# venetanji/videosd

Measured on AMD Instinct MI355X. Metric: frames/sec (whole node) + p50 per-frame latency, SD1.5 512x512 LCM 4-step, higher is better.
Workload: dtype f16 (fp32 accumulate); 1 GPU; 5 frames per launch x 4 launch lanes in flight (a stream's independent frames coalesced along GEMM M; the batch=1-per-launch figures of a --full run are fps_one_frame_per_launch and p50_latency_ms) of SD1.5 512x512 LCM 4-step img2img, every frame denoised independently, ControlNet-canny + TAESD (BASELINE configs[1], reference-faithful: the reference always runs ControlNet); frames_per_rank=411, frames_per_launch=5, launches_in_flight_per_gpu=4, kernel_launches_per_graph_replay=1430

## Files before the change

videosd_amd/csrc/attention.hip:

```cpp
#include <stdarg.h>
#include <stdlib.h>

#include <type_traits>

#include "common.h"

namespace {

struct AttnParams {
  const half_t* q;
  const half_t* k;
  const half_t* vt;
  half_t* out;
  int ldq, ldk, ldvt, ldo;
  int sq, sk, heads, d;
  float scale_log2;
  int causal;
  int k_brows, vt_bcols;
  VSD_CUT_FIELD
#ifdef VSD_ATTN_PROBE
  long long* probe;
#endif
};

#ifdef VSD_ATTN_PROBE
long long* g_probe = nullptr;
#define PROBE(I_)                                          \
  {                                                        \
    long long t_ = __builtin_readcyclecounter();           \
    pacc[I_] += t_ - plast;                                \
    plast = t_;                                            \
  }
#else
#define PROBE(I_)
#endif

constexpr float NEG_BIG = -1.0e30f;

#ifndef VSD_ATTN_PV_PRIO
#define VSD_ATTN_PV_PRIO 3
#endif

__device__ __forceinline__ float xhalf_max(float x) {
  auto r = __builtin_amdgcn_permlane32_swap(__float_as_uint(x), __float_as_uint(x), false, false);
  return fmaxf(__uint_as_float(r[0]), __uint_as_float(r[1]));
}

constexpr float LAZY_T = 5.0f;
template <int NQK, int NPV, int NW, int QB, int KSP, bool LAZY = false>
__device__ __forceinline__ void attention_body(const AttnParams& pp, const unsigned image) {
  VSD_CUT(VSD_CUT_ATTENTION, pp.cut)
  constexpr int NTG = 64 * NW;
  constexpr int KS = NQK * 16 + 8;
  constexpr int VS = 64 + 8;
  constexpr int DV = NPV * 32;
  constexpr int KTILE = 64 * KS, VTILE = DV * VS;
  constexpr int GROUP_HALFS = 2 * (KTILE + VTILE);
  constexpr int KCH = (64 * NQK * 2 + NTG - 1) / NTG;
  constexpr int VCH = (DV * 8 + NTG - 1) / NTG;
  constexpr int MERGE_FLOATS = KSP > 1 ? NW * QB * (NPV * 16 + 2) * 64 : 0;
  constexpr int SMEM_HALFS = (KSP * GROUP_HALFS > 2 * MERGE_FLOATS) ? KSP * GROUP_HALFS : 2 * MERGE_FLOATS;
  __shared__ __attribute__((aligned(16))) half_t smem[SMEM_HALFS];

  AttnParams p = pp;
  {
    const size_t b = image;
    p.q += b * p.sq * p.ldq;
    p.out += b * p.sq * p.ldo;
    p.k += b * p.k_brows * p.ldk;
    p.vt += b * p.vt_bcols;
  }
  const int tid = threadIdx.x;
  const int lane = tid & 63;
  const int wave = tid >> 6;
  const int grp = wave / NW;
  const int gwave = wave - grp * NW;
  const int gtid = tid - grp * NTG;
  const int lr = lane & 31;
  const int lh = lane >> 5;
  const int head = blockIdx.x;
  const int qblk = blockIdx.y;
  const int q0 = qblk * (32 * NW * QB) + gwave * (32 * QB);
  const int d = p.d;
  const int dch = d >> 3;
  half_t* Ks = smem + grp * GROUP_HALFS;
  half_t* Vs = Ks + 2 * KTILE;

  for (int i = tid; i < KSP * GROUP_HALFS / 8; i += NTG * KSP) reinterpret_cast<u32x4*>(smem)[i] = (u32x4){0u, 0u, 0u, 0u};
  const bool ones_row = d < DV;

  unsigned kg[KCH];
  int kl[KCH], krow[KCH];
#pragma unroll
  for (int i = 0; i < KCH; ++i) {
    int c = gtid + i * NTG;
    bool ok = c < 64 * dch;
    int kr = ok ? c / dch : 0, kc = ok ? c - kr * dch : 0;
    krow[i] = ok ? kr : 1 << 28;
    kg[i] = ok ? (unsigned)(kr * p.ldk + head * d + kc * 8) : 0u;
    kl[i] = kr * KS + kc * 8;
  }
  unsigned vg[VCH];
  int vl[VCH];
  bool vok[VCH];
#pragma unroll
  for (int i = 0; i < VCH; ++i) {
    int c = gtid + i * NTG;
    vok[i] = c < d * 8;
    int vr = vok[i] ? c >> 3 : 0, vc = c & 7;
    vg[i] = vok[i] ? (unsigned)((head * d + vr) * p.ldvt + vc * 8) : 0u;
    vl[i] = vr * VS + (vc >> 1) * 16 + (vc & 1) * 4;
  }
  u32x4 kreg[2][KCH], vreg[2][VCH];
#define ATT_LOAD_K(SET_, KEY0_)                                                                     \
  {                                                                                                 \
    const half_t* kb_ = p.k + (size_t)(KEY0_) * p.ldk;                                              \
    if ((KEY0_) + 64 <= p.sk) {                                                                     \
      _Pragma("unroll") for (int i = 0; i < KCH; ++i) kreg[SET_][i] = *reinterpret_cast<const u32x4*>(kb_ + kg[i]); \
    } else {                                                                                        \
      _Pragma("unroll") for (int i = 0; i < KCH; ++i) {                                             \
        const bool ok = (KEY0_) + krow[i] < p.sk;                                                   \
        kreg[SET_][i] = *reinterpret_cast<const u32x4*>(ok ? kb_ + kg[i] : p.k);                    \
      }                                                                                             \
    }                                                                                               \
  }
#define ATT_LOAD_V(SET_, KEY0_)                                                                     \
  {                                                                                                 \
    const half_t* vb_ = p.vt + (KEY0_);                                                             \
    _Pragma("unroll") for (int i = 0; i < VCH; ++i) vreg[SET_][i] = *reinterpret_cast<const u32x4*>(vb_ + vg[i]); \
  }
#define ATT_STORE_K(SET_, BUF_)                                                                     \
  {                                                                                                 \
    _Pragma("unroll") for (int i = 0; i < KCH; ++i)                                                 \
      if (krow[i] < 64) *reinterpret_cast<u32x4*>(Ks + (BUF_) * KTILE + kl[i]) = kreg[SET_][i];     \
  }
#define ATT_STORE_V(SET_, BUF_)                                                                     \
  {                                                                                                 \
    _Pragma("unroll") for (int i = 0; i < VCH; ++i)                                                 \
      if (vok[i]) {                                                                                 \
        half_t* dst = Vs + (BUF_) * VTILE + vl[i];                                                  \
        *reinterpret_cast<u32x2*>(dst) = (u32x2){vreg[SET_][i][0], vreg[SET_][i][1]};               \
        *reinterpret_cast<u32x2*>(dst + 8) = (u32x2){vreg[SET_][i][2], vreg[SET_][i][3]};           \
      }                                                                                             \
  }
#define ATT_LOAD(SET_, KEY0_) { ATT_LOAD_K(SET_, KEY0_) ATT_LOAD_V(SET_, KEY0_) }
#define ATT_STORE(SET_, BUF_) { ATT_STORE_K(SET_, BUF_) ATT_STORE_V(SET_, BUF_) }

  half8 qf[QB][NQK];
  int qrow[QB];
  bool qvalid[QB];
#pragma unroll
  for (int qb = 0; qb < QB; ++qb) {
    qrow[qb] = q0 + 32 * qb + lr;
    qvalid[qb] = qrow[qb] < p.sq;
#pragma unroll
    for (int ks = 0; ks < NQK; ++ks) {
      int doff = ks * 16 + lh * 8;
      half8 v = (half8){0, 0, 0, 0, 0, 0, 0, 0};
      if (qvalid[qb] && doff < d) {
        v = *reinterpret_cast<const half8*>(p.q + (size_t)qrow[qb] * p.ldq + head * d + doff);
#pragma unroll
        for (int j = 0; j < 8; ++j) v[j] = (half_t)((float)v[j] * p.scale_log2);
      }
      qf[qb][ks] = v;
    }
  }

  f32x16 o[QB][NPV];
  float m_run[QB], l_run[QB];
#pragma unroll
  for (int qb = 0; qb < QB; ++qb) {
    m_run[qb] = NEG_BIG;
    l_run[qb] = 0.f;
#pragma unroll
    for (int i = 0; i < NPV; ++i)
#pragma unroll
      for (int r = 0; r < 16; ++r) o[qb][i][r] = 0.f;
  }

  [[maybe_unused]] bool lazy_first = true;
  if constexpr (LAZY) {
#pragma unroll
    for (int qb = 0; qb < QB; ++qb) m_run[qb] = 0.f;
  }
  int sk_end = p.sk;
  if (p.causal) sk_end = min(p.sk, qblk * (32 * NW * QB) + 32 * NW * QB);
  const int ntiles = (sk_end + 63) / 64;
  const int niter = (ntiles + KSP - 1) / KSP;

  auto slot_key0 = [&](int j) { return (j * KSP + grp) * 64; };
  auto slot_ok = [&](int j) { return j * KSP + grp < ntiles; };
#ifdef VSD_ATTN_PROBE
  long long pacc[8] = {0, 0, 0, 0, 0, 0, 0, 0};
  long long plast = __builtin_readcyclecounter();
#endif
  auto qk_tile = [&](const int buf, f32x16 (&s)[QB][2]) __attribute__((always_inline)) {
      const half_t* Kb = Ks + buf * KTILE;
#pragma unroll
      for (int kb = 0; kb < 2; ++kb)
#pragma unroll
        for (int qb = 0; qb < QB; ++qb)
#pragma unroll
          for (int r = 0; r < 16; ++r) s[qb][kb][r] = 0.f;
#pragma unroll
      for (int ks = 0; ks < NQK; ++ks) {
#pragma unroll
        for (int kb = 0; kb < 2; ++kb) {
          half8 kf = *reinterpret_cast<const half8*>(Kb + (kb * 32 + lr) * KS + ks * 16 + lh * 8);
#pragma unroll
          for (int qb = 0; qb < QB; ++qb) s[qb][kb] = __builtin_amdgcn_mfma_f32_32x32x16_f16(kf, qf[qb][ks], s[qb][kb], 0, 0, 0);
        }
      }
      PROBE(1)
      __builtin_amdgcn_s_setprio(0);
  };
  auto softmax_pv = [&](const int buf, const int key0, auto masked, f32x16 (&s)[QB][2]) __attribute__((always_inline)) {
      const half_t* Vb = Vs + buf * VTILE;
      if constexpr (decltype(masked)::value) {
#pragma unroll
        for (int qb = 0; qb < QB; ++qb)
#pragma unroll
          for (int kb = 0; kb < 2; ++kb)
#pragma unroll
            for (int r = 0; r < 16; ++r) {
              int key = key0 + kb * 32 + (r & 3) + 8 * (r >> 2) + 4 * lh;
              bool ok = key < p.sk && (!p.causal || key <= qrow[qb]);
              if (!ok) s[qb][kb][r] = NEG_BIG;
            }
      }
      if constexpr (LAZY) {
        float mx[QB];
        bool need = false;
#pragma unroll
        for (int qb = 0; qb < QB; ++qb) {
          float v = NEG_BIG;
#pragma unroll
          for (int kb = 0; kb < 2; ++kb)
#pragma unroll
            for (int r = 0; r < 16; ++r) v = fmaxf(v, s[qb][kb][r]);
          mx[qb] = xhalf_max(v);
          need = need || mx[qb] > LAZY_T;
        }
        const bool moved = __builtin_amdgcn_ballot_w64(need) != 0;
        if (lazy_first || moved) {
#pragma unroll
          for (int qb = 0; qb < QB; ++qb) {
            const bool mine = lazy_first || mx[qb] > LAZY_T;
            float m_new = mine ? fminf(fmaxf(m_run[qb] + mx[qb], -60000.f), 60000.f) : m_run[qb];
            m_new = (float)(half_t)m_new;
            const float delta = m_new - m_run[qb];
            const float alpha = __builtin_amdgcn_exp2f(-delta);
#pragma unroll
            for (int kb = 0; kb < 2; ++kb)
#pragma unroll
              for (int r = 0; r < 16; ++r) s[qb][kb][r] = __builtin_amdgcn_exp2f(s[qb][kb][r] - delta);
            if (!lazy_first) {
#pragma unroll
              for (int i = 0; i < NPV; ++i)
#pragma unroll
                for (int r = 0; r < 16; ++r) o[qb][i][r] *= alpha;
            }
            m_run[qb] = m_new;
            if (lh == 1) qf[qb][NQK - 1][0] = (half_t)(-m_new);
          }
          lazy_first = false;
        } else {
#pragma unroll
          for (int qb = 0; qb < QB; ++qb)
#pragma unroll
            for (int kb = 0; kb < 2; ++kb)
#pragma unroll
              for (int r = 0; r < 16; ++r) s[qb][kb][r] = __builtin_amdgcn_exp2f(s[qb][kb][r]);
        }
      } else {
      bool grew_any = false;
      float alpha[QB];
#pragma unroll
      for (int qb = 0; qb < QB; ++qb) {
        float mx = NEG_BIG;
#pragma unroll
        for (int kb = 0; kb < 2; ++kb)
#pragma unroll
          for (int r = 0; r < 16; ++r) mx = fmaxf(mx, s[qb][kb][r]);
        mx = xhalf_max(mx);
        const float m_new = fmaxf(m_run[qb], mx);
        grew_any = grew_any || (m_new > m_run[qb]);
        alpha[qb] = __builtin_amdgcn_exp2f(m_run[qb] - m_new);
        m_run[qb] = m_new;
        if (ones_row) {
#pragma unroll
          for (int kb = 0; kb < 2; ++kb)
#pragma unroll
            for (int r = 0; r < 16; ++r) s[qb][kb][r] = __builtin_amdgcn_exp2f(s[qb][kb][r] - m_new);
        } else {
          float psum = 0.f;
#pragma unroll
          for (int kb = 0; kb < 2; ++kb)
#pragma unroll
            for (int r = 0; r < 16; ++r) {
              float e = __builtin_amdgcn_exp2f(s[qb][kb][r] - m_new);
              s[qb][kb][r] = e;
              psum += e;
            }
          l_run[qb] = l_run[qb] * alpha[qb] + psum;
        }
      }
      if (__builtin_amdgcn_ballot_w64(grew_any) != 0) {
#pragma unroll
        for (int qb = 0; qb < QB; ++qb)
#pragma unroll
          for (int i = 0; i < NPV; ++i)
#pragma unroll
            for (int r = 0; r < 16; ++r) o[qb][i][r] *= alpha[qb];
      }
      }

      PROBE(2)
      __builtin_amdgcn_s_setprio(VSD_ATTN_PV_PRIO);
#pragma unroll
      for (int kb = 0; kb < 2; ++kb) {
#pragma unroll
        for (int st = 0; st < 2; ++st) {
          half8 pf[QB];
#pragma unroll
          for (int qb = 0; qb < QB; ++qb)
#pragma unroll
            for (int j = 0; j < 8; ++j) pf[qb][j] = (half_t)s[qb][kb][8 * st + j];
#pragma unroll
          for (int db = 0; db < NPV; ++db) {
            half8 vf = *reinterpret_cast<const half8*>(Vb + (db * 32 + lr) * VS + kb * 32 + 16 * st + 8 * lh);
#pragma unroll
            for (int qb = 0; qb < QB; ++qb) o[qb][db] = __builtin_amdgcn_mfma_f32_32x32x16_f16(vf, pf[qb], o[qb][db], 0, 0, 0);
          }
        }
      }
      PROBE(3)
  };
  auto run_softmax_pv = [&](int j, const int buf, f32x16 (&s)[QB][2]) __attribute__((always_inline)) {
    const int key0 = slot_key0(j);
    if ((key0 + 64 > p.sk) || p.causal) softmax_pv(buf, key0, std::true_type{}, s);
    else softmax_pv(buf, key0, std::false_type{}, s);
  };

  if (slot_ok(0)) ATT_LOAD(0, slot_key0(0))
  if (slot_ok(1)) ATT_LOAD(1, slot_key0(1))
  __syncthreads();
  if (ones_row && gtid < 2 * 64) Vs[(gtid >> 6) * VTILE + (DV - 1) * VS + (gtid & 63)] = (half_t)1.0f;
  if (LAZY && gtid < 2 * 64) Ks[(gtid >> 6) * KTILE + (gtid & 63) * KS + d] = (half_t)1.0f;
  if (slot_ok(0)) ATT_STORE(0, 0)
  __syncthreads();
  auto run_tile = [&](int j) __attribute__((always_inline)) {
    f32x16 s[QB][2];
    qk_tile(j & 1, s);
    run_softmax_pv(j, j & 1, s);
  };
  for (int it = 0; it < niter; it += 2) {
    if (slot_ok(it + 2)) ATT_LOAD(0, slot_key0(it + 2))
    PROBE(0)
    if (slot_ok(it)) run_tile(it);
    if (slot_ok(it + 1)) ATT_STORE(1, 1)
    PROBE(4)
    __syncthreads();
    PROBE(5)
    if (it + 1 < niter) {
      if (slot_ok(it + 3)) ATT_LOAD(1, slot_key0(it + 3))
      PROBE(0)
      if (slot_ok(it + 1)) run_tile(it + 1);
      if (slot_ok(it + 2)) ATT_STORE(0, 0)
      PROBE(4)
    }
    __syncthreads();
    PROBE(5)
  }
#ifdef VSD_ATTN_PROBE
  if (p.probe && blockIdx.x == 0 && blockIdx.y == 0 && image == 0 && tid == 0)
    for (int i = 0; i < 8; ++i) p.probe[i] = pacc[i];
#endif
#undef ATT_LOAD
#undef ATT_STORE
#undef ATT_LOAD_K
#undef ATT_LOAD_V
#undef ATT_STORE_K
#undef ATT_STORE_V

  if constexpr (KSP > 1) {
    constexpr int PER_WAVE = QB * (NPV * 16 + 2) * 64;
    float* mg = reinterpret_cast<float*>(smem) + gwave * PER_WAVE + lane;
    if (grp == 1) {
#pragma unroll
      for (int qb = 0; qb < QB; ++qb) {
        float* b = mg + qb * (NPV * 16 + 2) * 64;
        b[0] = (LAZY && lazy_first) ? NEG_BIG : m_run[qb];
        b[64] = l_run[qb];
#pragma unroll
        for (int i = 0; i < NPV; ++i)
#pragma unroll
          for (int r = 0; r < 16; ++r) b[(2 + i * 16 + r) * 64] = o[qb][i][r];
      }
    }
    __syncthreads();
    if (grp != 0) return;
#pragma unroll
    for (int qb = 0; qb < QB; ++qb) {
      const float* b = mg + qb * (NPV * 16 + 2) * 64;
      const float m1 = b[0], l1 = b[64];
      const float m = fmaxf(m_run[qb], m1);
      const float a0 = __builtin_amdgcn_exp2f(m_run[qb] - m), a1 = __builtin_amdgcn_exp2f(m1 - m);
      l_run[qb] = l_run[qb] * a0 + l1 * a1;
#pragma unroll
      for (int i = 0; i < NPV; ++i)
#pragma unroll
        for (int r = 0; r < 16; ++r) o[qb][i][r] = o[qb][i][r] * a0 + b[(2 + i * 16 + r) * 64] * a1;
    }
  }

#pragma unroll
  for (int qb = 0; qb < QB; ++qb) {
    float l_tot;
    if (ones_row) {
      const float mine = o[qb][NPV - 1][15];
      const float other = __shfl_xor(mine, 32);
      l_tot = lh ? mine : other;
    } else {
      l_tot = l_run[qb] + __shfl_xor(l_run[qb], 32);
    }
    const float inv = 1.0f / l_tot;
    if (qvalid[qb]) {
      half_t* orow = p.out + (size_t)qrow[qb] * p.ldo + head * d;
#pragma unroll
      for (int db = 0; db < NPV; ++db)
#pragma unroll
        for (int g = 0; g < 4; ++g) {
          int dd = db * 32 + 8 * g + 4 * lh;
          if (dd < d) {
            half4 v;
#pragma unroll
            for (int j = 0; j < 4; ++j) v[j] = (half_t)(o[qb][db][4 * g + j] * inv);
            *reinterpret_cast<half4*>(orow + dd) = v;
          }
        }
    }
  }
}

template <int NQK, int NPV, int NW, int QB, int KSP, bool LAZY = false>
__global__ __launch_bounds__(64 * NW * KSP) void attention_kernel(const AttnParams pp) {
  attention_body<NQK, NPV, NW, QB, KSP, LAZY>(pp, blockIdx.z);
}
template <int NQK, int NPV, int NW, int QB, int KSP>
__global__ __launch_bounds__(64 * NW * KSP) __attribute__((amdgpu_waves_per_eu(3))) void attention_lazy_kernel(const AttnParams pp) {
  attention_body<NQK, NPV, NW, QB, KSP, true>(pp, blockIdx.z);
}
template <int NQK, int NPV, int NW, int QB, int KSP>
__global__ __launch_bounds__(64 * NW * KSP) __attribute__((amdgpu_waves_per_eu(3))) void attention_lazy_pair_kernel(const Pair<AttnParams> g) {
  const unsigned nb = gridDim.z >> 1, which = blockIdx.z >= nb;
  attention_body<NQK, NPV, NW, QB, KSP, true>(g.p[which], blockIdx.z - which * nb);
}
template <int NQK, int NPV, int NW, int QB, int KSP, bool LAZY = false>
__global__ __launch_bounds__(64 * NW * KSP) void attention_pair_kernel(const Pair<AttnParams> g) {
  const unsigned nb = gridDim.z >> 1, which = blockIdx.z >= nb;
  attention_body<NQK, NPV, NW, QB, KSP, LAZY>(g.p[which], blockIdx.z - which * nb);
}

struct AttnShape {
  int nw, qb, ksp;
};

template <int NQK, int NPV, int NW, int QB, int KSP>
void launch_one(vsd_ctx* ctx, const AttnParams& p, int batch, hipStream_t s) {
  dim3 grid(p.heads, (p.sq + 32 * NW * QB - 1) / (32 * NW * QB), batch);
  if constexpr (NQK == 3 && NPV == 2) {
    static const bool off = getenv("VSD_ATTN_NO_LAZY") != nullptr;
    if (p.d == 40 && !p.causal && !off) {
      if constexpr (NW == 4 && KSP == 1)
        launch_pairable(ctx, attention_lazy_kernel<NQK, NPV, NW, QB, KSP>, attention_lazy_pair_kernel<NQK, NPV, NW, QB, KSP>, grid, dim3(64 * NW * KSP), 0, s, p);
      else
        launch_pairable(ctx, attention_kernel<NQK, NPV, NW, QB, KSP, true>, attention_pair_kernel<NQK, NPV, NW, QB, KSP, true>, grid, dim3(64 * NW * KSP), 0, s, p);
      return;
    }
  }
  launch_pairable(ctx, attention_kernel<NQK, NPV, NW, QB, KSP>, attention_pair_kernel<NQK, NPV, NW, QB, KSP>, grid, dim3(64 * NW * KSP), 0, s, p);
}

template <int NQK, int NPV>
void launch_attn(vsd_ctx* ctx, const AttnParams& p, AttnShape sh, int batch, hipStream_t s) {
  constexpr bool SMALL = NPV <= 3;
  if constexpr (SMALL) {
    if (sh.ksp == 2) return launch_one<NQK, NPV, 4, 1, 2>(ctx, p, batch, s);
  }
  if (sh.nw == 2) return launch_one<NQK, NPV, 2, 1, 1>(ctx, p, batch, s);
  return launch_one<NQK, NPV, 4, 1, 1>(ctx, p, batch, s);
}

}

#ifdef VSD_ATTN_PROBE
extern "C" void vsd_attn_set_probe(void* buf) { g_probe = (long long*)buf; }
#endif

extern "C" int vsd_attention(vsd_ctx* ctx, const void* q, int ldq, const void* k, int ldk, const void* vt, int ldvt,
                             void* out, int ldo, int sq, int sk, int heads, int d, float scale, int causal,
                             void* stream) {
  return vsd_attention_batched(ctx, q, ldq, k, ldk, vt, ldvt, out, ldo, sq, sk, heads, d, scale, causal, 1, 0, 0, stream);
}

extern "C" int vsd_attention_batched(vsd_ctx* ctx, const void* q, int ldq, const void* k, int ldk, const void* vt, int ldvt,
                                     void* out, int ldo, int sq, int sk, int heads, int d, float scale, int causal,
                                     int batch, int k_batch_rows, int vt_batch_cols, void* stream) {
  if (!ctx) return VSD_ERR_ARG;
#ifdef VSD_PROBE
  { static const bool skip = getenv("VSD_SKIP_ATTN") != nullptr; if (skip) return VSD_OK; }
#endif
  if (batch < 1 || batch > 65535 || k_batch_rows < 0 || vt_batch_cols < 0 || vt_batch_cols % 8)
    return vsd_fail(ctx, VSD_ERR_ARG, "attention: batch=%d k_batch_rows=%d vt_batch_cols=%d", batch, k_batch_rows, vt_batch_cols);
  if (!q || !k || !vt || !out) return vsd_fail(ctx, VSD_ERR_ARG, "attention: null pointer");
  if (d % 8 || d < 8 || d > 160) return vsd_fail(ctx, VSD_ERR_ARG, "attention: head_dim %d unsupported", d);
  if (sq <= 0 || sk <= 0 || heads <= 0) return vsd_fail(ctx, VSD_ERR_ARG, "attention: empty problem");
  if (ldq % 8 || ldk % 8 || ldvt % 8 || ldo % 4 || ldvt < (batch - 1) * vt_batch_cols + ((sk + 63) / 64) * 64)
    return vsd_fail(ctx, VSD_ERR_ARG, "attention: bad leading dimensions (ldvt=%d must cover round_up(sk=%d,64))", ldvt, sk);
  AttnParams p;
  p.q = (const half_t*)q; p.k = (const half_t*)k; p.vt = (const half_t*)vt; p.out = (half_t*)out;
  p.ldq = ldq; p.ldk = ldk; p.ldvt = ldvt; p.ldo = ldo;
  p.sq = sq; p.sk = sk; p.heads = heads; p.d = d;
  p.scale_log2 = scale * 1.4426950408889634f;
  p.causal = causal;
  p.k_brows = k_batch_rows; p.vt_bcols = vt_batch_cols;
  VSD_CUT_SET(p)
#ifdef VSD_ATTN_PROBE
  p.probe = g_probe;
#endif
  hipStream_t s = (hipStream_t)stream;
  LaunchScope ls(ctx, s, VSD_FAM_ATTENTION, 4.0 * sq * (double)sk * heads * d * batch);
  const int nqk = (d + 15) / 16;
  const long wgs = (long)((sq + 127) / 128) * heads * batch;
  AttnShape sh = {4, 1, 1};
  const int ntiles = (sk + 63) / 64;
  if (d <= 96 && !causal && ntiles >= 8 && wgs <= 256) sh.ksp = 2;
  if (sh.ksp == 1 && wgs < 64) sh.nw = 2;
  if (const char* e = getenv("VSD_ATTN_SHAPE")) {
    int a = 4, b = 1, c = 1;
    if (sscanf(e, "%d,%d,%d", &a, &b, &c) == 3) {
      sh.nw = a == 2 ? 2 : 4;
      sh.qb = 1;
      (void)b;
      sh.ksp = (c == 2 && d <= 96) ? 2 : 1;
    }
  }
  if (nqk <= 1) launch_attn<1, 1>(ctx, p, sh, batch, s);
  else if (nqk == 2) launch_attn<2, 1>(ctx, p, sh, batch, s);
  else if (nqk == 3) launch_attn<3, 2>(ctx, p, sh, batch, s);
  else if (nqk == 4) launch_attn<4, 2>(ctx, p, sh, batch, s);
  else if (nqk == 5) launch_attn<5, 3>(ctx, p, sh, batch, s);
  else if (nqk == 6) launch_attn<6, 3>(ctx, p, sh, batch, s);
  else if (nqk <= 8) launch_attn<8, 4>(ctx, p, sh, batch, s);
  else launch_attn<10, 5>(ctx, p, sh, batch, s);
  return ls.finish();
}
```

Before: 142.4 frames/s.

## Add register-resident short-key attention kernel for cross-attention with few keys

Adds a specialised attention kernel for short key sequences (sk<=96, d<=64, heads<=8), such as the text-conditioning cross-attention with 77 keys. Each wave keeps all K and V fragments for one head in registers, computes the full softmax in a single pass with no online rescaling, and loops over several 32-row query blocks. Each 512-thread block covers all heads, and the next query block is prefetched while the current one is computed. It is chosen automatically when there are enough query blocks to fill the GPU, and trades higher register use and a separate code path for removing repeated K/V loads and the flash-attention bookkeeping.

```diff
diff --git a/videosd_amd/csrc/attention.hip b/videosd_amd/csrc/attention.hip
--- a/videosd_amd/csrc/attention.hip
+++ b/videosd_amd/csrc/attention.hip
@@ -460,6 +460,195 @@
 __global__ __launch_bounds__(64 * NW * KSP) void attention_pair_kernel(const Pair<AttnParams> g) {
   const unsigned nb = gridDim.z >> 1, which = blockIdx.z >= nb;
   attention_body<NQK, NPV, NW, QB, KSP, LAZY>(g.p[which], blockIdx.z - which * nb);
+}
+
+struct ShortParams {
+  AttnParams a;
+  int nsub;
+  int trips;
+};
+
+template <int NQK, int NPV, int NKB>
+__device__ __forceinline__ void attention_short_body(const ShortParams& sp, const unsigned image) {
+  VSD_CUT(VSD_CUT_ATTENTION, sp.a.cut)
+  constexpr int DV = NPV * 32;
+  AttnParams p = sp.a;
+  {
+    const size_t b = image;
+    p.q += b * p.sq * p.ldq;
+    p.out += b * p.sq * p.ldo;
+    p.k += b * p.k_brows * p.ldk;
+    p.vt += b * p.vt_bcols;
+  }
+  const int lane = threadIdx.x & 63;
+  const int wave = threadIdx.x >> 6;
+  const int lr = lane & 31;
+  const int lh = lane >> 5;
+  const int sub = wave / p.heads;
+  const int head = wave - sub * p.heads;
+  if (sub >= sp.nsub) return;
+  const int d = p.d;
+  const bool ones_row = d < DV;
+
+  half8 kf[NKB][NQK];
+#pragma unroll
+  for (int kb = 0; kb < NKB; ++kb)
+#pragma unroll
+    for (int ks = 0; ks < NQK; ++ks) {
+      const int key = kb * 32 + lr, doff = ks * 16 + lh * 8;
+      half8 v = (half8){0, 0, 0, 0, 0, 0, 0, 0};
+      if (key < p.sk && doff < d) v = *reinterpret_cast<const half8*>(p.k + (size_t)key * p.ldk + head * d + doff);
+      kf[kb][ks] = v;
+    }
+  half8 vf[NPV][NKB][2];
+#pragma unroll
+  for (int db = 0; db < NPV; ++db) {
+    const int dd = db * 32 + lr;
+    const half_t* vrow = p.vt + (size_t)(head * d + (dd < d ? dd : 0)) * p.ldvt;
+#pragma unroll
+    for (int kb = 0; kb < NKB; ++kb)
+#pragma unroll
+      for (int st = 0; st < 2; ++st) {
+        const int key0 = kb * 32 + 16 * st + 8 * lh;
+        u32x4 raw = (u32x4){0u, 0u, 0u, 0u};
+        if (dd < d) {
+          half8 v = *reinterpret_cast<const half8*>(vrow + key0);
+          if (kb == NKB - 1) {
+#pragma unroll
+            for (int j = 0; j < 8; ++j)
+              if (key0 + j >= p.sk) v[j] = (half_t)0.0f;
+          }
+          raw = __builtin_bit_cast(u32x4, v);
+        } else if (ones_row && dd == DV - 1) {
+          raw = (u32x4){0x3c003c00u, 0x3c003c00u, 0x3c003c00u, 0x3c003c00u};
+        }
+        const auto s0 = __builtin_amdgcn_permlane32_swap(raw[0], raw[2], false, false);
+        const auto s1 = __builtin_amdgcn_permlane32_swap(raw[1], raw[3], false, false);
+        const half8 v = __builtin_bit_cast(half8, ((u32x4){s0[0], s1[0], s0[1], s1[1]}));
+        vf[db][kb][st] = v;
+      }
+  }
+  const int tail = p.sk - (NKB - 1) * 32 - 4 * lh;
+
+  const int blk0 = blockIdx.x * (sp.nsub * sp.trips) + sub;
+  const int nblk = (p.sq + 31) >> 5;
+  auto load_q = [&](int blk, half8 (&raw)[NQK]) __attribute__((always_inline)) {
+    const int row = blk * 32 + lr;
+#pragma unroll
+    for (int ks = 0; ks < NQK; ++ks) {
+      const int doff = ks * 16 + lh * 8;
+      half8 v = (half8){0, 0, 0, 0, 0, 0, 0, 0};
+      if (row < p.sq && doff < d) v = *reinterpret_cast<const half8*>(p.q + (size_t)row * p.ldq + head * d + doff);
+      raw[ks] = v;
+    }
+  };
+  half8 qraw[NQK];
+  if (blk0 < nblk) load_q(blk0, qraw);
+  for (int t = 0; t < sp.trips; ++t) {
+    const int blk = blk0 + t * sp.nsub;
+    if (blk >= nblk) break;
+    half8 qf[NQK];
+#pragma unroll
+    for (int ks = 0; ks < NQK; ++ks)
+#pragma unroll
+      for (int j = 0; j < 8; ++j) qf[ks][j] = (half_t)((float)qraw[ks][j] * p.scale_log2);
+    if (t + 1 < sp.trips && blk + sp.nsub < nblk) load_q(blk + sp.nsub, qraw);
+
+    f32x16 s[NKB];
+#pragma unroll
+    for (int kb = 0; kb < NKB; ++kb)
+#pragma unroll
+      for (int r = 0; r < 16; ++r) s[kb][r] = 0.f;
+#pragma unroll
+    for (int ks = 0; ks < NQK; ++ks)
+#pragma unroll
+      for (int kb = 0; kb < NKB; ++kb) s[kb] = __builtin_amdgcn_mfma_f32_32x32x16_f16(kf[kb][ks], qf[ks], s[kb], 0, 0, 0);
+#pragma unroll
+    for (int r = 0; r < 16; ++r)
+      if ((r & 3) + 8 * (r >> 2) >= tail) s[NKB - 1][r] = NEG_BIG;
+    float mx = NEG_BIG;
+#pragma unroll
+    for (int kb = 0; kb < NKB; ++kb)
+#pragma unroll
+      for (int r = 0; r < 16; ++r) mx = fmaxf(mx, s[kb][r]);
+    mx = xhalf_max(mx);
+    float psum = 0.f;
+#pragma unroll
+    for (int kb = 0; kb < NKB; ++kb)
+#pragma unroll
+      for (int r = 0; r < 16; ++r) {
+        s[kb][r] = __builtin_amdgcn_exp2f(s[kb][r] - mx);
+        if (!ones_row) psum += s[kb][r];
+      }
+    f32x16 o[NPV];
+#pragma unroll
+    for (int db = 0; db < NPV; ++db)
+#pragma unroll
+      for (int r = 0; r < 16; ++r) o[db][r] = 0.f;
+#pragma unroll
+    for (int kb = 0; kb < NKB; ++kb)
+#pragma unroll
+      for (int st = 0; st < 2; ++st) {
+        half8 pf;
+#pragma unroll
+        for (int j = 0; j < 8; ++j) pf[j] = (half_t)s[kb][8 * st + j];
+#pragma unroll
+        for (int db = 0; db < NPV; ++db) o[db] = __builtin_amdgcn_mfma_f32_32x32x16_f16(vf[db][kb][st], pf, o[db], 0, 0, 0);
+      }
+    float l_tot;
+    if (ones_row) {
+      const float mine = o[NPV - 1][15];
+      const float other = __shfl_xor(mine, 32);
+      l_tot = lh ? mine : other;
+    } else {
+      l_tot = psum + __shfl_xor(psum, 32);
+    }
+    const float inv = 1.0f / l_tot;
+    const int qrow = blk * 32 + lr;
+    half_t* orow = p.out + (size_t)qrow * p.ldo + head * d;
+#pragma unroll
+    for (int db = 0; db < NPV; ++db)
+#pragma unroll
+      for (int g = 0; g < 4; g += 2) {
+        half4 lo, hi;
+#pragma unroll
+        for (int j = 0; j < 4; ++j) {
+          lo[j] = (half_t)(o[db][4 * g + j] * inv);
+          hi[j] = (half_t)(o[db][4 * g + 4 + j] * inv);
+        }
+        const u32x2 a = __builtin_bit_cast(u32x2, lo), b = __builtin_bit_cast(u32x2, hi);
+        const auto s0 = __builtin_amdgcn_permlane32_swap(a[0], b[0], false, false);
+        const auto s1 = __builtin_amdgcn_permlane32_swap(a[1], b[1], false, false);
+        const int dd = db * 32 + 8 * (g + lh);
+        if (qrow < p.sq && dd < d) *reinterpret_cast<u32x4*>(orow + dd) = (u32x4){s0[0], s1[0], s0[1], s1[1]};
+      }
+  }
+}
+
+template <int NQK, int NPV, int NKB>
+__global__ __launch_bounds__(512) void attention_short_kernel(const ShortParams sp) {
+  attention_short_body<NQK, NPV, NKB>(sp, blockIdx.z);
+}
+template <int NQK, int NPV, int NKB>
+__global__ __launch_bounds__(512) void attention_short_pair_kernel(const Pair<ShortParams> g) {
+  const unsigned nb = gridDim.z >> 1, which = blockIdx.z >= nb;
+  attention_short_body<NQK, NPV, NKB>(g.p[which], blockIdx.z - which * nb);
+}
+
+template <int NQK, int NPV>
+void launch_short(vsd_ctx* ctx, const AttnParams& p, int batch, hipStream_t s) {
+  ShortParams sp;
+  sp.a = p;
+  sp.nsub = 8 / p.heads;
+  const long blocks = (long)batch * ((p.sq + 31) / 32);
+  const long slots = (long)(ctx->num_cus > 0 ? ctx->num_cus : 256) * sp.nsub;
+  sp.trips = (int)((blocks + slots - 1) / slots);
+  const int rows = 32 * sp.nsub * sp.trips;
+  dim3 grid((p.sq + rows - 1) / rows, 1, batch);
+  const int nkb = (p.sk + 31) / 32;
+  if (nkb == 1) launch_pairable(ctx, attention_short_kernel<NQK, NPV, 1>, attention_short_pair_kernel<NQK, NPV, 1>, grid, dim3(512), 0, s, sp);
+  else if (nkb == 2) launch_pairable(ctx, attention_short_kernel<NQK, NPV, 2>, attention_short_pair_kernel<NQK, NPV, 2>, grid, dim3(512), 0, s, sp);
+  else launch_pairable(ctx, attention_short_kernel<NQK, NPV, 3>, attention_short_pair_kernel<NQK, NPV, 3>, grid, dim3(512), 0, s, sp);
 }
 
 struct AttnShape {
@@ -537,7 +726,21 @@
   const int ntiles = (sk + 63) / 64;
   if (d <= 96 && !causal && ntiles >= 8 && wgs <= 256) sh.ksp = 2;
   if (sh.ksp == 1 && wgs < 64) sh.nw = 2;
-  if (const char* e = getenv("VSD_ATTN_SHAPE")) {
+  const char* const shape_env = getenv("VSD_ATTN_SHAPE");
+  static const bool no_short = getenv("VSD_ATTN_NO_SHORT") != nullptr;
+  const bool short_fits = sk <= 96 && d <= 64 && heads <= 8 && !causal && ldo % 8 == 0 && ((uintptr_t)out & 15) == 0;
+  if (short_fits && !no_short) {
+    const bool asked = shape_env && !strcmp(shape_env, "short");
+    const long blocks = (long)batch * ((sq + 31) / 32), slots = (long)(ctx->num_cus > 0 ? ctx->num_cus : 256) * (8 / heads);
+    if (asked || (!shape_env && blocks > 2 * slots)) {
+      if (nqk <= 1) launch_short<1, 1>(ctx, p, batch, s);
+      else if (nqk == 2) launch_short<2, 1>(ctx, p, batch, s);
+      else if (nqk == 3) launch_short<3, 2>(ctx, p, batch, s);
+      else launch_short<4, 2>(ctx, p, batch, s);
+      return ls.finish();
+    }
+  }
+  if (const char* e = shape_env) {
     int a = 4, b = 1, c = 1;
     if (sscanf(e, "%d,%d,%d", &a, &b, &c) == 3) {
       sh.nw = a == 2 ? 2 : 4;
```

After: 142.6 frames/s (median of 3 runs). No clear change (+0.1%).
